# phonism/genrec

Hardware: AMD Instinct MI355X
Metric: train_samples_per_s (higher is better)
Workload: dtype bf16; 1 GPU; model=tiger-amazon-beauty, global_batch=256, seq_len=61, parallelism=dp1, hip_graph=True

## Files before the change

csrc/bindings.cpp:

```cpp
#include <torch/extension.h>

namespace genrec {

std::vector<torch::Tensor> rms_norm_fwd(torch::Tensor x, torch::Tensor w,
                                        double eps, bool t5_style);
std::vector<torch::Tensor> rms_norm_bwd(torch::Tensor dy, torch::Tensor x,
                                        torch::Tensor w, torch::Tensor inv_rms,
                                        bool t5_style);
std::vector<torch::Tensor> l2norm_fwd(torch::Tensor x, double eps);
torch::Tensor l2norm_bwd(torch::Tensor dy, torch::Tensor x,
                         torch::Tensor inv_norm, double eps);

std::vector<torch::Tensor> attn_fwd(
    torch::Tensor q, torch::Tensor k, torch::Tensor v,
    c10::optional<torch::Tensor> bias, c10::optional<torch::Tensor> key_pad,
    c10::optional<torch::Tensor> add_mask,
    c10::optional<torch::Tensor> query_mask,
    double scale, bool causal, int64_t act, double dropout_p, int64_t seed,
    c10::optional<torch::Tensor> seed_dev);
std::vector<torch::Tensor> attn_bwd(
    torch::Tensor dout, torch::Tensor q, torch::Tensor k, torch::Tensor v,
    torch::Tensor p_saved, torch::Tensor drop_mask,
    c10::optional<torch::Tensor> query_mask,
    double scale, int64_t act, double dropout_p, int64_t seed,
    bool bias_grad, int64_t bias_dim);

std::vector<torch::Tensor> attn_fwd_mfma(
    torch::Tensor q, torch::Tensor k, torch::Tensor v,
    c10::optional<torch::Tensor> bias, c10::optional<torch::Tensor> key_pad,
    c10::optional<torch::Tensor> add_mask,
    c10::optional<torch::Tensor> query_mask,
    double scale, bool causal, int64_t act, double dropout_p, int64_t seed,
    c10::optional<torch::Tensor> seed_dev,
    c10::optional<torch::Tensor> bias_bucket);
std::vector<torch::Tensor> attn_bwd_mfma(
    torch::Tensor dout, torch::Tensor q, torch::Tensor k, torch::Tensor v,
    torch::Tensor p_saved, torch::Tensor drop_mask,
    c10::optional<torch::Tensor> query_mask,
    double scale, int64_t act, double dropout_p, int64_t seed,
    bool bias_grad, int64_t bias_dim,
    c10::optional<torch::Tensor> bias_bucket, int64_t n_buckets);

std::vector<torch::Tensor> hstu_attn_fwd(
    torch::Tensor q, torch::Tensor k, torch::Tensor v,
    torch::Tensor pos_bucket, torch::Tensor pos_table,
    c10::optional<torch::Tensor> time_table,
    c10::optional<torch::Tensor> timestamps,
    c10::optional<torch::Tensor> key_pad);
std::vector<torch::Tensor> hstu_attn_bwd(
    torch::Tensor dout, torch::Tensor q, torch::Tensor k, torch::Tensor v,
    torch::Tensor s_saved, torch::Tensor pos_bucket,
    c10::optional<torch::Tensor> timestamps,
    int64_t n_pos, int64_t n_time);

std::vector<torch::Tensor> softmax_ce_fwd(torch::Tensor logits,
                                          torch::Tensor targets,
                                          int64_t ignore_index);
torch::Tensor softmax_ce_bwd(torch::Tensor dloss, torch::Tensor logits,
                             torch::Tensor targets, torch::Tensor lse,
                             torch::Tensor n_valid, int64_t ignore_index);
std::vector<torch::Tensor> lce_inplace(torch::Tensor logits,
                                       torch::Tensor targets,
                                       torch::Tensor inv_n,
                                       int64_t ignore_index, int64_t slices);
int64_t lce_pick_slices(int64_t R, int64_t V);

std::vector<torch::Tensor> sqdist_argmin(torch::Tensor x,
                                         torch::Tensor codebook);
torch::Tensor embedding_fwd(torch::Tensor weight, torch::Tensor indices);
torch::Tensor embedding_bwd(torch::Tensor dy, torch::Tensor indices,
                            int64_t num_weights, int64_t padding_idx);
std::vector<torch::Tensor> dropout_add_fwd(
    torch::Tensor x, torch::Tensor residual, double p, int64_t seed,
    c10::optional<torch::Tensor> seed_dev);
// ... 49 lines not shown
    torch::Tensor out, torch::Tensor lse,
    c10::optional<torch::Tensor> key_pad, double scale, bool causal);

torch::Tensor beam_attn_fwd(torch::Tensor q, torch::Tensor k_pre,
                            torch::Tensor v_pre,
                            c10::optional<torch::Tensor> pre_pad,
                            torch::Tensor k_suf, torch::Tensor v_suf,
                            torch::Tensor anc, int64_t t, double scale,
                            int64_t splits);
int64_t beam_attn_pick_splits(int64_t B, int64_t Hkv, int64_t rows,
                              int64_t Lp);

}

PYBIND11_MODULE(TORCH_EXTENSION_NAME, m) {
  m.def("rms_norm_fwd", &genrec::rms_norm_fwd, "fused RMSNorm forward");
  m.def("rms_norm_bwd", &genrec::rms_norm_bwd, "fused RMSNorm backward");
  m.def("l2norm_fwd", &genrec::l2norm_fwd, "fused L2Norm forward");
  m.def("l2norm_bwd", &genrec::l2norm_bwd, "fused L2Norm backward");
  m.def("attn_fwd", &genrec::attn_fwd, "fused attention forward");
  m.def("attn_bwd", &genrec::attn_bwd, "fused attention backward");
  m.def("attn_fwd_mfma", &genrec::attn_fwd_mfma, "MFMA attention forward",
        py::arg("q"), py::arg("k"), py::arg("v"), py::arg("bias"),
        py::arg("key_pad"), py::arg("add_mask"), py::arg("query_mask"),
        py::arg("scale"), py::arg("causal"), py::arg("act"),
        py::arg("dropout_p"), py::arg("seed"), py::arg("seed_dev"),
        py::arg("bias_bucket") = py::none());
  m.def("attn_bwd_mfma", &genrec::attn_bwd_mfma, "MFMA attention backward",
        py::arg("dout"), py::arg("q"), py::arg("k"), py::arg("v"),
        py::arg("p_saved"), py::arg("drop_mask"), py::arg("query_mask"),
        py::arg("scale"), py::arg("act"), py::arg("dropout_p"),
        py::arg("seed"), py::arg("bias_grad"), py::arg("bias_dim"),
        py::arg("bias_bucket") = py::none(),
        py::arg("n_buckets") = 0);
  m.def("hstu_attn_fwd", &genrec::hstu_attn_fwd, "HSTU fused attention fwd");
  m.def("hstu_attn_bwd", &genrec::hstu_attn_bwd, "HSTU fused attention bwd");
  m.def("softmax_ce_fwd", &genrec::softmax_ce_fwd, "fused CE forward");
  m.def("softmax_ce_bwd", &genrec::softmax_ce_bwd, "fused CE backward");
  m.def("lce_inplace", &genrec::lce_inplace,
        "in-place CE fwd+bwd over a logits chunk (lce_stats + lce_grad)",
        py::arg("logits"), py::arg("targets"), py::arg("inv_n"),
        py::arg("ignore_index"), py::arg("slices") = 0);
  m.def("lce_pick_slices", &genrec::lce_pick_slices,
        "column slices per row chosen for an [R, V] chunk");
  m.def("sqdist_argmin", &genrec::sqdist_argmin, "L2 dist + argmin");
  m.def("embedding_fwd", &genrec::embedding_fwd, "embedding gather");
  m.def("embedding_bwd", &genrec::embedding_bwd, "embedding scatter-add bwd");
  m.def("dropout_add_fwd", &genrec::dropout_add_fwd, "residual+dropout fwd");
  m.def("relu_dropout_fwd", &genrec::relu_dropout_fwd, "dropout(relu) fwd");
  m.def("plain_dropout_fwd", &genrec::plain_dropout_fwd,
        "graph-replay-safe plain dropout fwd");
  m.def("colsum", &genrec::colsum,
        "deterministic replay-safe column sum (bias grads)");
  m.def("chunk_sum", &genrec::chunk_sum,
        "small-row-count column sum (split-K dW partials)");
  m.def("layer_norm_fwd", &genrec::layer_norm_fwd, "fused LayerNorm fwd");
  m.def("layer_norm_bwd", &genrec::layer_norm_bwd, "fused LayerNorm bwd");
  m.def("dropout_fuse_bwd", &genrec::dropout_fuse_bwd, "fused dropout bwd");
  m.def("dropout_add_rms_norm_fwd", &genrec::dropout_add_rms_norm_fwd,
        "fused residual+dropout -> RMSNorm fwd -> (h, n, mask, inv_rms)");
  m.def("dropout_add_rms_norm_bwd", &genrec::dropout_add_rms_norm_bwd,
        "fused RMSNorm bwd + dh add + dropout bwd -> (t, dy, dw)");
  m.def("topk_hit_ranks", &genrec::topk_hit_ranks, "first-match ranks");
  m.def("fused_adamw", &genrec::fused_adamw,
        "fused flat AdamW step (device lr/scale/step scalars)");
  m.def("skinny_gemm", &genrec::skinny_gemm,
        "tall-skinny linear fwd GEMM (bf16, fp32 accum)");
// ... 19 lines not shown
```

csrc/kernels/attention_mfma.hip:

```cpp

#include <torch/extension.h>
#include <ATen/hip/HIPContext.h>

#include "../core/mfma_tile.h"

namespace genrec {

torch::Tensor colsum(torch::Tensor x);

template <bool IS_SILU>
__global__ void __launch_bounds__(256, 5)
attn_fwd_mfma_kernel(
    const __hip_bfloat16* __restrict__ q,
    const __hip_bfloat16* __restrict__ k,
    const __hip_bfloat16* __restrict__ v,
    const void* __restrict__ bias,
    const int* __restrict__ bias_bucket,
    const bool* __restrict__ key_pad,
    const float* __restrict__ add_mask,
    const float* __restrict__ query_mask,
    __hip_bfloat16* __restrict__ out,
    float* __restrict__ p_saved,
    unsigned char* __restrict__ drop_mask,
    const unsigned int* __restrict__ seed_dev,
    int B, int H, int Lq, int Lk, int D, int n_buckets,
    int64_t q_sb, int64_t q_sh, int64_t q_sl,
    int64_t k_sb, int64_t k_sh, int64_t k_sl,
    int64_t v_sb, int64_t v_sh, int64_t v_sl,
    int64_t o_sb, int64_t o_sh, int64_t o_sl,
    float scale, int bias_dim, bool bias_bf16, bool causal,
    float dropout_p, unsigned int seed, int q_tile) {
  if (seed_dev) seed += *seed_dev;
  const float* bias_f = reinterpret_cast<const float*>(bias);
  const __hip_bfloat16* bias_b = reinterpret_cast<const __hip_bfloat16*>(bias);
  const int bh = blockIdx.x;
  const int b = bh / H, h = bh % H;
  const int q0 = blockIdx.y * q_tile;

  extern __shared__ __attribute__((aligned(16))) char smem[];
  char* qs = smem;
  char* ks = qs + TILE * 128;
// ... 279 lines not shown
  float da[2][4], ad[2][4];
#pragma unroll
  for (int fi = 0; fi < 2; ++fi) {
#pragma unroll
    for (int r = 0; r < 4; ++r) {
      int i = strip + row_grp + r;
      int j = (fbase + fi) * 16 + col_base;
      bool ok = (i < Lq) && (j < Lk);
      float p = pv[fi][r];
      float m = 1.f;
      if (!IS_SILU && ok) {
        if (query_mask) m *= qm_v[r];
        if (dropout_p > 0.f) m *= dm_v[fi][r] ? inv_keep : 0.f;
      }
      da[fi][r] = ok ? acc[fi][r] * (IS_SILU ? 1.f : m) : 0.f;
      ad[fi][r] = IS_SILU ? (ok ? p * sigmoidf_dev(p) : 0.f) : p * m;
    }
  }

  float ds[2][4];
  if (IS_SILU) {
#pragma unroll
    for (int fi = 0; fi < 2; ++fi)
#pragma unroll
      for (int r = 0; r < 4; ++r) {
        float s = pv[fi][r];
        float sg = sigmoidf_dev(s);
        ds[fi][r] = da[fi][r] * sg * (1.f + s * (1.f - sg));
      }
  } else {
    float part[4];
#pragma unroll
    for (int r = 0; r < 4; ++r)
      part[r] = grp16_sum(da[0][r] * pv[0][r] + da[1][r] * pv[1][r]);
    if (col_base == 0) {
#pragma unroll
      for (int r = 0; r < 4; ++r)
        dotbuf[half * TILE + strip + row_grp + r] = part[r];
    }
    __syncthreads();
#pragma unroll
    for (int r = 0; r < 4; ++r) {
      float dot_r = dotbuf[strip + row_grp + r] +
                    dotbuf[TILE + strip + row_grp + r];
#pragma unroll
      for (int fi = 0; fi < 2; ++fi)
        ds[fi][r] = pv[fi][r] * (da[fi][r] - dot_r);
    }
  }

  const int i0 = strip + row_grp;
#pragma unroll
  for (int fi = 0; fi < 2; ++fi) {
    short4v dpack, apack;
#pragma unroll
    for (int r = 0; r < 4; ++r) {
      int i = i0 + r;
      int j = (fbase + fi) * 16 + col_base;
      float dval = (i < Lq && j < Lk) ? ds[fi][r] : 0.f;
      float aval = (i < Lq && j < Lk) ? ad[fi][r] : 0.f;
      dpack[r] = bf16_bits(dval * scale);
      apack[r] = bf16_bits(aval);
      if (ds_saved && i < Lq && j < Lk) {
        ds_saved[idx4(b, h, i, j, H, Lq, Lk)] = __float2bfloat16(dval);
      }
      if (dtab_partial && i < Lq && j < Lk) {
        atomicAdd(&tab_lds[bias_bucket[(int64_t)i * Lk + j]], dval);
// ... 32 lines not shown
              __float2bfloat16(accq[fi][r]);
        }
      }
    }
  }

  {
    float4v acck[2] = {{0.f, 0.f, 0.f, 0.f}, {0.f, 0.f, 0.f, 0.f}};
    float4v accv[2] = {{0.f, 0.f, 0.f, 0.f}, {0.f, 0.f, 0.f, 0.f}};
#pragma unroll
    for (int fi = 0; fi < 2; ++fi) {
      if (fbase + fi >= nfrag_d) break;
      for (int kk = 0; kk < TILE; kk += 32) {
        short8v a1 = frag_load<true>(dst, strip, kk, lane);
        short8v b1 = frag_load_tr(qs, kk, (fbase + fi) * 16, lane);
        acck[fi] = mfma_bf16(a1, b1, acck[fi]);
        short8v a2 = frag_load<true>(adt, strip, kk, lane);
        short8v b2 = frag_load_tr(dos, kk, (fbase + fi) * 16, lane);
        accv[fi] = mfma_bf16(a2, b2, accv[fi]);
      }
    }
#pragma unroll
    for (int fi = 0; fi < 2; ++fi) {
      if (fbase + fi >= nfrag_d) break;
#pragma unroll
      for (int r = 0; r < 4; ++r) {
        int j = strip + row_grp + r;
        int d = (fbase + fi) * 16 + col_base;
        if (j < Lk && d < D) {
          dk_out[(int64_t)b * dk_sb + h * dk_sh + j * dk_sl + d] =
              __float2bfloat16(acck[fi][r]);
          dv_out[(int64_t)b * dv_sb + h * dv_sh + j * dv_sl + d] =
              __float2bfloat16(accv[fi][r]);
        }
      }
    }
  }
}

constexpr int BS_CH = 16;

__global__ void batch_sum1_kernel(const __hip_bfloat16* __restrict__ in,
                                  float* __restrict__ tmp,
                                  int B, int64_t inner) {
  int64_t tid = (int64_t)blockIdx.x * blockDim.x + threadIdx.x;
  if (tid >= (int64_t)BS_CH * inner) return;
  int64_t j = tid % inner;
  int chunk = (int)(tid / inner);
  float acc = 0.f;
  for (int b = chunk; b < B; b += BS_CH)
    acc += to_f32(in[(int64_t)b * inner + j]);
  tmp[(int64_t)chunk * inner + j] = acc;
}

__global__ void batch_sum2_kernel(const float* __restrict__ tmp,
                                  float* __restrict__ out, int64_t inner) {
  int64_t j = (int64_t)blockIdx.x * blockDim.x + threadIdx.x;
  if (j >= inner) return;
  float acc = 0.f;
#pragma unroll
  for (int r = 0; r < BS_CH; ++r) acc += tmp[(int64_t)r * inner + j];
  out[j] = acc;
}


std::vector<torch::Tensor> attn_fwd_mfma(
    torch::Tensor q, torch::Tensor k, torch::Tensor v,
    c10::optional<torch::Tensor> bias, c10::optional<torch::Tensor> key_pad,
    c10::optional<torch::Tensor> add_mask,
    c10::optional<torch::Tensor> query_mask,
    double scale, bool causal, int64_t act, double dropout_p, int64_t seed,
    c10::optional<torch::Tensor> seed_dev,
    c10::optional<torch::Tensor> bias_bucket) {
  TORCH_CHECK(q.scalar_type() == torch::kBFloat16);
  const int B = q.size(0), H = q.size(1), Lq = q.size(2), D = q.size(3);
  const int Lk = k.size(2);
  TORCH_CHECK(Lk <= TILE && D <= TILE && D % 32 == 0);
  TORCH_CHECK(q.stride(3) == 1 && k.stride(3) == 1 && v.stride(3) == 1,
              "attn_fwd_mfma: innermost (D) stride must be 1");
  auto out = torch::empty_like(q);
  auto p_saved = torch::empty({B, H, Lq, Lk},
                              q.options().dtype(torch::kFloat32));
  torch::Tensor dmask;
  if (dropout_p > 0) {
    dmask = torch::empty({B, H, Lq, Lk}, q.options().dtype(torch::kUInt8));
  } else {
    dmask = torch::empty({0}, q.options().dtype(torch::kUInt8));
  }
  torch::Tensor bias_c, bucket_c;
  int bias_dim = 0;
  bool bias_bf16 = false;
  int n_buckets = 0;
  if (bias_bucket.has_value()) {
    TORCH_CHECK(bias.has_value() &&
                bias->scalar_type() == torch::kFloat32);
    bias_c = bias->contiguous();
    bucket_c = bias_bucket->to(torch::kInt32).contiguous();
    n_buckets = (int)(bias_c.numel() / H);
  } else if (bias.has_value()) {
    TORCH_CHECK(bias->scalar_type() == torch::kFloat32 ||
                bias->scalar_type() == torch::kBFloat16);
    bias_c = bias->contiguous();
    bias_dim = bias_c.dim();
    bias_bf16 = bias_c.scalar_type() == torch::kBFloat16;
  }
  torch::Tensor am_f, qm_f;
  if (add_mask.has_value()) am_f = add_mask->to(torch::kFloat32).contiguous();
  if (query_mask.has_value())
    qm_f = query_mask->to(torch::kFloat32).contiguous();

  const int q_tile = TILE;
  dim3 block(256);
  dim3 grid(B * H, (Lq + q_tile - 1) / q_tile);
  size_t smem = 4 * TILE * 128;
  auto stream = at::cuda::getCurrentHIPStream();

#define LAUNCH_FWD_MFMA(SILU)                                                  \
  hipLaunchKernelGGL((attn_fwd_mfma_kernel<SILU>), grid, block, smem, stream,  \
      reinterpret_cast<const __hip_bfloat16*>(q.data_ptr()),                   \
      reinterpret_cast<const __hip_bfloat16*>(k.data_ptr()),                   \
      reinterpret_cast<const __hip_bfloat16*>(v.data_ptr()),                   \
      (bias_dim || n_buckets) ? bias_c.data_ptr() : nullptr,                   \
      n_buckets ? bucket_c.data_ptr<int>() : nullptr,                          \
      key_pad.has_value() ? key_pad->data_ptr<bool>() : nullptr,               \
      add_mask.has_value() ? am_f.data_ptr<float>() : nullptr,                 \
      query_mask.has_value() ? qm_f.data_ptr<float>() : nullptr,               \
      reinterpret_cast<__hip_bfloat16*>(out.data_ptr()),                       \
      p_saved.data_ptr<float>(),                                               \
      dropout_p > 0 ? dmask.data_ptr<unsigned char>() : nullptr,               \
      seed_dev.has_value()                                                     \
          ? reinterpret_cast<const unsigned int*>(seed_dev->data_ptr())        \
          : nullptr,                                                           \
      B, H, Lq, Lk, D, n_buckets,                                              \
      q.stride(0), q.stride(1), q.stride(2),                                   \
      k.stride(0), k.stride(1), k.stride(2),                                   \
      v.stride(0), v.stride(1), v.stride(2),                                   \
      out.stride(0), out.stride(1), out.stride(2),                             \
      (float)scale, bias_dim, bias_bf16, causal,                               \
      (float)dropout_p, (unsigned int)seed, q_tile)

  if (act == 0) LAUNCH_FWD_MFMA(false);
  else LAUNCH_FWD_MFMA(true);
#undef LAUNCH_FWD_MFMA
  return {out, p_saved, dmask};
}

std::vector<torch::Tensor> attn_bwd_mfma(
    torch::Tensor dout, torch::Tensor q, torch::Tensor k, torch::Tensor v,
    torch::Tensor p_saved, torch::Tensor drop_mask,
    c10::optional<torch::Tensor> query_mask,
    double scale, int64_t act, double dropout_p, int64_t seed,
    bool bias_grad, int64_t bias_dim,
    c10::optional<torch::Tensor> bias_bucket, int64_t n_buckets) {
  (void)seed;
  const int B = q.size(0), H = q.size(1), Lq = q.size(2), D = q.size(3);
  const int Lk = k.size(2);
  TORCH_CHECK(Lq <= TILE && Lk <= TILE && D % 32 == 0);
  TORCH_CHECK(dout.stride(3) == 1 && q.stride(3) == 1 && k.stride(3) == 1 &&
                  v.stride(3) == 1,
              "attn_bwd_mfma: innermost (D) stride must be 1");
  auto dq = torch::empty_like(q);
  auto dk = torch::empty_like(k);
  auto dv = torch::empty_like(v);
  torch::Tensor ds_saved, bucket_c, dtab_partial;
  __hip_bfloat16* ds_ptr = nullptr;
  const bool table_mode = bias_grad && bias_bucket.has_value();
  if (table_mode) {
    bucket_c = bias_bucket->to(torch::kInt32).contiguous();
    dtab_partial = torch::empty({(int64_t)B * H, n_buckets},
                                q.options().dtype(torch::kFloat32));
  } else if (bias_grad) {
    ds_saved = torch::empty({B, H, Lq, Lk},
                            q.options().dtype(torch::kBFloat16));
    ds_ptr = reinterpret_cast<__hip_bfloat16*>(ds_saved.data_ptr());
  }
  torch::Tensor qm_f;
  if (query_mask.has_value())
    qm_f = query_mask->to(torch::kFloat32).contiguous();
  dim3 block(512);
  dim3 grid(B * H);
  size_t smem = 6 * TILE * 128 + 2 * TILE * sizeof(float)
      + (table_mode ? (size_t)n_buckets * sizeof(float) : 0);
  auto stream = at::cuda::getCurrentHIPStream();

#define LAUNCH_BWD_DS(SILU)                                                    \
  hipLaunchKernelGGL((attn_bwd_ds_kernel<SILU>), grid, block, smem, stream,    \
      reinterpret_cast<const __hip_bfloat16*>(dout.data_ptr()),                \
      reinterpret_cast<const __hip_bfloat16*>(q.data_ptr()),                   \
      reinterpret_cast<const __hip_bfloat16*>(k.data_ptr()),                   \
      reinterpret_cast<const __hip_bfloat16*>(v.data_ptr()),                   \
      p_saved.data_ptr<float>(),                                               \
      query_mask.has_value() ? qm_f.data_ptr<float>() : nullptr,               \
      dropout_p > 0 ? drop_mask.data_ptr<unsigned char>() : nullptr,           \
      reinterpret_cast<__hip_bfloat16*>(dq.data_ptr()),                        \
      reinterpret_cast<__hip_bfloat16*>(dk.data_ptr()),                        \
      reinterpret_cast<__hip_bfloat16*>(dv.data_ptr()), ds_ptr,                \
      table_mode ? bucket_c.data_ptr<int>() : nullptr,                         \
      table_mode ? dtab_partial.data_ptr<float>() : nullptr,                   \
      (int)n_buckets,                                                          \
      B, H, Lq, Lk, D,                                                         \
      dout.stride(0), dout.stride(1), dout.stride(2),                          \
      q.stride(0), q.stride(1), q.stride(2),                                   \
      k.stride(0), k.stride(1), k.stride(2),                                   \
      v.stride(0), v.stride(1), v.stride(2),                                   \
      dq.stride(0), dq.stride(1), dq.stride(2),                                \
      dk.stride(0), dk.stride(1), dk.stride(2),                                \
      dv.stride(0), dv.stride(1), dv.stride(2),                                \
      (float)scale, (float)dropout_p)

  if (act == 0) LAUNCH_BWD_DS(false);
  else LAUNCH_BWD_DS(true);
#undef LAUNCH_BWD_DS

  torch::Tensor dbias;
  if (table_mode) {
    dbias = colsum(dtab_partial.view({B, (int64_t)H * n_buckets}));
  } else if (bias_grad) {
    if (bias_dim == 3) {
      const int64_t inner = (int64_t)H * Lq * Lk;
      dbias = torch::empty({H, Lq, Lk},
                           q.options().dtype(torch::kFloat32));
      auto tmp = torch::empty({16, inner},
                              q.options().dtype(torch::kFloat32));
      dim3 rblock(256);
      dim3 rgrid1((unsigned)((16 * inner + 255) / 256));
      hipLaunchKernelGGL(batch_sum1_kernel, rgrid1, rblock, 0, stream,
          reinterpret_cast<const __hip_bfloat16*>(ds_saved.data_ptr()),
          tmp.data_ptr<float>(), B, inner);
      dim3 rgrid2((unsigned)((inner + 255) / 256));
      hipLaunchKernelGGL(batch_sum2_kernel, rgrid2, rblock, 0, stream,
          tmp.data_ptr<float>(), dbias.data_ptr<float>(), inner);
    } else {
      dbias = ds_saved.to(torch::kFloat32);
    }
  } else {
    dbias = torch::empty({0}, q.options().dtype(torch::kFloat32));
  }
  return {dq, dk, dv, dbias};
}

}
```

genrec_amd/modules/transformer.py:

```python

from __future__ import annotations

import math
import os
from typing import Optional

import torch
from torch import Tensor, nn

from genrec_amd import ops
from genrec_amd.ops.linear import SplitKLinear
from genrec_amd.modules.norms import RMSNorm, T5RMSNorm


def relative_position_bucket(relative_positions: Tensor, num_buckets: int = 32,
                             max_distance: int = 128,
                             bidirectional: bool = True) -> Tensor:
    ret = -relative_positions
    if bidirectional:
        num_buckets //= 2
        sign = (ret < 0).long()
        ret = ret.abs()
    else:
        ret = torch.clamp_min(ret, 0)
# ... 61 lines not shown
        return ops.embedding(self.rel_bias.weight, idx).view(
            self.n_heads, q_len, k_len)

    def _bucket_map(self, q_len: int, k_len: int, device) -> Tensor:
        key = ("bm", q_len, k_len, str(device))
        bm = self._bucket_cache.get(key)
        if bm is None:
            ctx = torch.arange(q_len, device=device)[:, None]
            mem = torch.arange(k_len, device=device)[None, :]
            bm = relative_position_bucket(
                mem - ctx, self.num_relative_buckets, self.max_distance,
                bidirectional=True).to(torch.int32).contiguous()
            self._bucket_cache[key] = bm
        return bm

    def _split(self, x: Tensor) -> Tensor:
        b, l, _ = x.shape
        return x.view(b, l, self.n_heads, self.head_dim).transpose(1, 2)

    def forward(self, query: Tensor, key: Optional[Tensor] = None,
                value: Optional[Tensor] = None,
                attn_mask: Optional[Tensor] = None,
                key_padding_mask: Optional[Tensor] = None,
                kv_cache: Optional[dict] = None) -> Tensor:
        if self.is_cross_attention:
            if kv_cache is not None and "k" in kv_cache:
                k, v = kv_cache["k"], kv_cache["v"]
            else:
                k, v = self._split(self.k(key)), self._split(self.v(value))
                if kv_cache is not None:
                    kv_cache["k"], kv_cache["v"] = k, v
        else:
            qkv = self.qkv(query)
            q_flat, k, v = qkv.chunk(3, dim=-1)
            k, v = self._split(k), self._split(v)
            if kv_cache is not None:
                if "k" in kv_cache:
                    k = torch.cat([kv_cache["k"], k], dim=2)
                    v = torch.cat([kv_cache["v"], v], dim=2)
                kv_cache["k"], kv_cache["v"] = k, v
            q = self._split(q_flat)
            return self._attend(q, k, v, attn_mask, key_padding_mask)
        q = self._split(self.q(query))
        return self._attend(q, k, v, attn_mask, key_padding_mask)

    def _attend(self, q: Tensor, k: Tensor, v: Tensor,
                attn_mask: Optional[Tensor],
                key_padding_mask: Optional[Tensor]) -> Tensor:

        bias = None
        bias_table = bias_bucket = None
        if self.rel_bias is not None:
            if os.environ.get("GENREC_ATTN_TABLE_BIAS", "0") == "1" \
                    and q.is_cuda:
                bias_table = self.rel_bias.weight.view(-1)
                bm = self._bucket_map(k.size(2), k.size(2), q.device)
                if q.size(2) != k.size(2):
                    bm = bm[k.size(2) - q.size(2):, :].contiguous()
                bias_bucket = bm
            else:
                bias = self.compute_bias(k.size(2), k.size(2), q.device)
                if q.size(2) != k.size(2):
                    bias = bias[:, k.size(2) - q.size(2):, :]

        out = ops.t5_attention(
            q, k, v, bias, key_padding_mask, attn_mask, self.scale,
# ... 175 lines not shown
```

genrec_amd/ops/__init__.py:

```python

from __future__ import annotations

import os

import torch

_EXT = None
_EXT_ERR: Exception | None = None


def _load_ext():
    global _EXT, _EXT_ERR
    if _EXT is not None or _EXT_ERR is not None:
        return _EXT
    try:
        from genrec_amd import _C

        _EXT = _C
    except ImportError as e:
        _EXT_ERR = e
        _EXT = None
    return _EXT


# ... 3 lines not shown
        raise RuntimeError(
            "genrec_amd HIP extension (genrec_amd._C) is not built. "
            "Run `python setup.py build_ext --inplace` (gfx950). "
            f"Import error: {_EXT_ERR}"
        )
    return m


def has_ext() -> bool:
    return _load_ext() is not None


def _force_eager() -> bool:
    return os.environ.get("GENREC_AMD_FORCE_EAGER", "0") == "1"


def use_hip(*tensors: torch.Tensor) -> bool:
    if _force_eager():
        return False
    if not tensors or not tensors[0].is_cuda:
        return False
    ext()
    return True


from genrec_amd.ops import eager
from genrec_amd.ops.norms import (
    layer_norm, rms_norm, l2norm_op, swish_layer_norm,
)
from genrec_amd.ops.attention import (
    fused_attention,
    sasrec_attention,
    t5_attention,
    hstu_pointwise_attention,
    hstu_fused_attention,
    gqa_flash_attention,
    beam_decode_attention,
    beam_decode_supported,
)
from genrec_amd.ops.quantize import residual_quantize_step
from genrec_amd.ops.losses import (
    softmax_ce, tied_softmax_ce, summed_ce, linear_cross_entropy,
)
from genrec_amd.ops.metrics import topk_hit_ranks
from genrec_amd.ops.embedding import embedding
from genrec_amd.ops.fused import (
    dropout_add, dropout_add_rms_norm, plain_dropout, relu_dropout,
)

__all__ = [
    "ext",
    "has_ext",
    "use_hip",
    "eager",
    "rms_norm",
    "l2norm_op",
    "swish_layer_norm",
    "layer_norm",
    "fused_attention",
    "sasrec_attention",
    "t5_attention",
    "hstu_pointwise_attention",
    "hstu_fused_attention",
    "gqa_flash_attention",
    "beam_decode_attention",
    "beam_decode_supported",
    "residual_quantize_step",
    "softmax_ce",
    "tied_softmax_ce",
    "summed_ce",
    "linear_cross_entropy",
    "topk_hit_ranks",
    "embedding",
    "dropout_add",
    "dropout_add_rms_norm",
    "plain_dropout",
    "relu_dropout",
]
```

genrec_amd/ops/attention.py:

```python

from __future__ import annotations

import os
from typing import Optional

import torch
from torch import Tensor

from genrec_amd.ops import eager

_ACT_SOFTMAX = 0
_ACT_SILU = 1


def _kernel_available(name: str, *tensors: Tensor) -> bool:
    from genrec_amd import ops

    if not ops.use_hip(*tensors):
        return False
    return hasattr(ops.ext(), name)


_seed_counters = {}
_call_salt = [0]
# ... 43 lines not shown
        out, probs, dmask = fwd(
            q, k, v, bias, key_pad_mask, additive_mask, query_mask,
            scale, causal, act, dropout_p if training else 0.0, seed,
            seed_dev,
        )
        ctx.use_mfma = use_mfma
        ctx.save_for_backward(q, k, v, probs, dmask,
                              query_mask if query_mask is not None else torch.empty(0))
        ctx.meta = (scale, causal, act, dropout_p if training else 0.0, seed,
                    bias is not None and bias.requires_grad,
                    bias.dim() if bias is not None else 0,
                    bias.dtype if bias is not None else None)
        return out

    @staticmethod
    def backward(ctx, dout):
        from genrec_amd import ops

        q, k, v, probs, dmask, query_mask = ctx.saved_tensors
        (scale, causal, act, dropout_p, seed, bias_grad, bias_dim,
         bias_dtype) = ctx.meta
        bwd = ops.ext().attn_bwd_mfma if ctx.use_mfma else ops.ext().attn_bwd
        if not (ctx.use_mfma and dout.stride(-1) == 1):
            dout = dout.contiguous()
        dq, dk, dv, dbias = bwd(
            dout, q, k, v, probs, dmask,
            query_mask if query_mask.numel() else None,
            scale, act, dropout_p, seed, bias_grad, bias_dim,
        )
        if bias_grad and dbias.dtype != bias_dtype:
            dbias = dbias.to(bias_dtype)
        return (dq, dk, dv, dbias if bias_grad else None,
                None, None, None, None, None, None, None, None)


class _FusedAttnTableBiasFn(torch.autograd.Function):

    @staticmethod
    def forward(ctx, q, k, v, bias_table, bias_bucket, key_pad_mask,
                additive_mask, query_mask, scale, causal, dropout_p,
                training):
        from genrec_amd import ops

        q = q if q.stride(-1) == 1 else q.contiguous()
        k = k if k.stride(-1) == 1 else k.contiguous()
        v = v if v.stride(-1) == 1 else v.contiguous()
        table_f = bias_table.float()
        seed_dev = None
        seed = 0
        if dropout_p > 0 and training:
            seed = _call_seed()
            seed_dev = _seed_counter(q.device)
        out, probs, dmask = ops.ext().attn_fwd_mfma(
            q, k, v, table_f, key_pad_mask, additive_mask, query_mask,
            scale, causal, 0, dropout_p if training else 0.0, seed,
            seed_dev, bias_bucket)
        ctx.save_for_backward(
            q, k, v, probs, dmask,
            query_mask if query_mask is not None else torch.empty(0),
            bias_bucket)
        ctx.meta = (scale, dropout_p if training else 0.0,
                    bias_table.requires_grad,
                    bias_table.numel() // q.size(1), bias_table.dtype)
        return out

    @staticmethod
# ... 331 lines not shown
```

Baseline: 54330 samples/s.

## Add small-Lq wave-per-head attention kernels and packed QKV self-attention path

```diff
diff --git a/csrc/bindings.cpp b/csrc/bindings.cpp
--- a/csrc/bindings.cpp
+++ b/csrc/bindings.cpp
@@ -39,7 +39,10 @@
     c10::optional<torch::Tensor> query_mask,
     double scale, int64_t act, double dropout_p, int64_t seed,
     bool bias_grad, int64_t bias_dim,
-    c10::optional<torch::Tensor> bias_bucket, int64_t n_buckets);
+    c10::optional<torch::Tensor> bias_bucket, int64_t n_buckets,
+    c10::optional<torch::Tensor> dqkv_out);
+std::string attn_mfma_path(int64_t Lq, int64_t Lk, int64_t D, int64_t act,
+                           bool table_mode, bool backward);
 
 std::vector<torch::Tensor> hstu_attn_fwd(
     torch::Tensor q, torch::Tensor k, torch::Tensor v,
@@ -155,7 +158,14 @@
         py::arg("scale"), py::arg("act"), py::arg("dropout_p"),
         py::arg("seed"), py::arg("bias_grad"), py::arg("bias_dim"),
         py::arg("bias_bucket") = py::none(),
-        py::arg("n_buckets") = 0);
+        py::arg("n_buckets") = 0,
+        py::arg("dqkv_out") = py::none());
+  m.def("attn_mfma_path", &genrec::attn_mfma_path,
+        "kernel family attn_fwd_mfma (attn_bwd_mfma: backward=True) runs "
+        "for a shape: "
+        "\"smallq\" or \"tile64\"",
+        py::arg("Lq"), py::arg("Lk"), py::arg("D"), py::arg("act") = 0,
+        py::arg("table_mode") = false, py::arg("backward") = false);
   m.def("hstu_attn_fwd", &genrec::hstu_attn_fwd, "HSTU fused attention fwd");
   m.def("hstu_attn_bwd", &genrec::hstu_attn_bwd, "HSTU fused attention bwd");
   m.def("softmax_ce_fwd", &genrec::softmax_ce_fwd, "fused CE forward");
diff --git a/csrc/kernels/attention_mfma.hip b/csrc/kernels/attention_mfma.hip
--- a/csrc/kernels/attention_mfma.hip
+++ b/csrc/kernels/attention_mfma.hip
@@ -7,6 +7,11 @@
 namespace genrec {
 
 torch::Tensor colsum(torch::Tensor x);
+
+__device__ __forceinline__ float jac_dot2(float a0, float b0, float a1,
+                                          float b1) {
+  return __builtin_fmaf(a0, b0, a1 * b1);
+}
 
 template <bool IS_SILU>
 __global__ void __launch_bounds__(256, 5)
@@ -352,7 +357,7 @@
     float part[4];
 #pragma unroll
     for (int r = 0; r < 4; ++r)
-      part[r] = grp16_sum(da[0][r] * pv[0][r] + da[1][r] * pv[1][r]);
+      part[r] = grp16_sum(jac_dot2(da[0][r], pv[0][r], da[1][r], pv[1][r]));
     if (col_base == 0) {
 #pragma unroll
       for (int r = 0; r < 4; ++r)
@@ -451,6 +456,485 @@
               __float2bfloat16(acck[fi][r]);
           dv_out[(int64_t)b * dv_sb + h * dv_sh + j * dv_sl + d] =
               __float2bfloat16(accv[fi][r]);
+        }
+      }
+    }
+  }
+}
+
+constexpr int SQ_HEADS = 2;
+constexpr int SQ_LQ = 16;
+constexpr int SQ_BWD_LK = 16;
+
+static inline int sq_rows32(int L) { return (L + 31) & ~31; }
+static inline size_t sq_fwd_lds(int Lk) {
+  return (size_t)(16 + 2 * sq_rows32(Lk)) * 128;
+}
+static inline size_t sq_bwd_lds(int Lk) {
+  return (size_t)(64 + 2 * sq_rows32(Lk)) * 128;
+}
+
+__device__ __forceinline__ void wave_lds_sync() {
+  __builtin_amdgcn_fence(__ATOMIC_ACQ_REL, "wavefront");
+  __builtin_amdgcn_wave_barrier();
+}
+
+template <int NF>
+__global__ void __launch_bounds__(64 * SQ_HEADS)
+attn_fwd_smallq_kernel(
+    const __hip_bfloat16* __restrict__ q,
+    const __hip_bfloat16* __restrict__ k,
+    const __hip_bfloat16* __restrict__ v,
+    const void* __restrict__ bias,
+    const bool* __restrict__ key_pad,
+    const float* __restrict__ add_mask,
+    const float* __restrict__ query_mask,
+    __hip_bfloat16* __restrict__ out,
+    float* __restrict__ p_saved,
+    unsigned char* __restrict__ drop_mask,
+    const unsigned int* __restrict__ seed_dev,
+    int B, int H, int Lq, int Lk, int D,
+    int64_t q_sb, int64_t q_sh, int64_t q_sl,
+    int64_t k_sb, int64_t k_sh, int64_t k_sl,
+    int64_t v_sb, int64_t v_sh, int64_t v_sl,
+    int64_t o_sb, int64_t o_sh, int64_t o_sl,
+    float scale, int bias_dim, bool bias_bf16, bool causal,
+    float dropout_p, unsigned int seed) {
+  const int lane = threadIdx.x & 63;
+  const int wid = __builtin_amdgcn_readfirstlane(threadIdx.x >> 6);
+  const int bh = blockIdx.x * SQ_HEADS + wid;
+  if (bh >= B * H) return;
+  if (seed_dev) seed += *seed_dev;
+  const float* bias_f = reinterpret_cast<const float*>(bias);
+  const __hip_bfloat16* bias_b = reinterpret_cast<const __hip_bfloat16*>(bias);
+  const int b = bh / H, h = bh % H;
+  constexpr int nf = NF;
+  constexpr int kr = (NF + 1) / 2 * 32;
+
+  extern __shared__ __attribute__((aligned(16))) char smem[];
+  char* qs = smem + (size_t)wid * (16 + 2 * kr) * 128;
+  char* ks = qs + 16 * 128;
+  char* vs = ks + kr * 128;
+  char* pt = ks;
+
+  const int col_base = frag_col(lane);
+  const int row_grp = frag_row0(lane);
+
+  const int st_row = lane >> 3;
+  const int st_d0 = (lane & 7) * 8;
+  short8v qq8[2], kk8[kr / 8], vv8[kr / 8];
+#pragma unroll
+  for (int c = 0; c < 2; ++c) {
+    int row = c * 8 + st_row;
+    qq8[c] = load8(q, (int64_t)b * q_sb + h * q_sh + row * q_sl + st_d0,
+                   row < Lq && st_d0 < D);
+  }
+#pragma unroll
+  for (int c = 0; c < kr / 8; ++c) {
+    int row = c * 8 + st_row;
+    kk8[c] = load8(k, (int64_t)b * k_sb + h * k_sh + row * k_sl + st_d0,
+                   row < Lk && st_d0 < D);
+    vv8[c] = load8(v, (int64_t)b * v_sb + h * v_sh + row * v_sl + st_d0,
+                   row < Lk && st_d0 < D);
+  }
+
+  float bias_v[4][4], am_v[4][4];
+  bool kp_v[4];
+#pragma unroll
+  for (int f = 0; f < 4; ++f) {
+    int j = f * 16 + col_base;
+    kp_v[f] = (key_pad && f < nf && j < Lk) ? key_pad[(int64_t)b * Lk + j] : false;
+#pragma unroll
+    for (int r = 0; r < 4; ++r) {
+      int i = row_grp + r;
+      bool ok = (f < nf) && (i < Lq) && (j < Lk);
+      float bv = 0.f, av = 0.f;
+      if (ok) {
+        if (bias_dim) {
+          int64_t bi = (bias_dim == 3) ? ((int64_t)h * Lq + i) * Lk + j
+                                       : idx4(b, h, i, j, H, Lq, Lk);
+          bv = bias_bf16 ? to_f32(bias_b[bi]) : bias_f[bi];
+        }
+        if (add_mask) av = add_mask[(int64_t)i * Lk + j];
+      }
+      bias_v[f][r] = bv;
+      am_v[f][r] = av;
+    }
+  }
+
+#pragma unroll
+  for (int c = 0; c < 2; ++c)
+    tile_store(qs, c * 8 + st_row, st_d0, qq8[c]);
+#pragma unroll
+  for (int c = 0; c < kr / 8; ++c) {
+    if (c * 8 < nf * 16) tile_store(ks, c * 8 + st_row, st_d0, kk8[c]);
+    tile_store<true>(vs, c * 8 + st_row, st_d0, vv8[c]);
+  }
+  wave_lds_sync();
+
+  const float inv_keep = dropout_p > 0.f ? 1.0f / (1.0f - dropout_p) : 1.0f;
+
+  float4v acc[4] = {{0.f, 0.f, 0.f, 0.f}, {0.f, 0.f, 0.f, 0.f},
+                    {0.f, 0.f, 0.f, 0.f}, {0.f, 0.f, 0.f, 0.f}};
+#pragma unroll
+  for (int f = 0; f < 4; ++f) {
+    if (f >= nf) break;
+    for (int kk = 0; kk < D; kk += 32) {
+      short8v a = frag_load(qs, 0, kk, lane);
+      short8v bfr = frag_load(ks, f * 16, kk, lane);
+      acc[f] = mfma_bf16(a, bfr, acc[f]);
+    }
+  }
+
+  float s_val[4][4];
+#pragma unroll
+  for (int f = 0; f < 4; ++f) {
+#pragma unroll
+    for (int r = 0; r < 4; ++r) {
+      int i = row_grp + r;
+      int j = f * 16 + col_base;
+      float s = acc[f][r];
+      bool ok = (f < nf) && (i < Lq) && (j < Lk);
+      if (ok) {
+        s *= scale;
+        if (bias_dim) s += bias_v[f][r];
+        if (causal && j > i) s = NEG_BIG;
+        if (kp_v[f]) s = NEG_BIG;
+        if (add_mask) s += am_v[f][r];
+      } else {
+        s = -INFINITY;
+      }
+      s_val[f][r] = s;
+    }
+  }
+
+  float p_val[4][4];
+#pragma unroll
+  for (int r = 0; r < 4; ++r) {
+    float m = grp16_max(fmaxf(fmaxf(s_val[0][r], s_val[1][r]),
+                              fmaxf(s_val[2][r], s_val[3][r])));
+    float sum = 0.f;
+#pragma unroll
+    for (int f = 0; f < 4; ++f) {
+      float e = (s_val[f][r] == -INFINITY) ? 0.f
+                                           : __expf(s_val[f][r] - m);
+      p_val[f][r] = e;
+      sum += e;
+    }
+    sum = grp16_sum(sum);
+    float inv = (sum > 0.f) ? 1.0f / sum : 0.f;
+#pragma unroll
+    for (int f = 0; f < 4; ++f) p_val[f][r] *= inv;
+  }
+
+  wave_lds_sync();
+
+#pragma unroll
+  for (int f = 0; f < 4; ++f) {
+    if (f * 16 >= kr) break;
+    short4v ppack;
+#pragma unroll
+    for (int r = 0; r < 4; ++r) {
+      int i = row_grp + r;
+      int j = f * 16 + col_base;
+      float p = p_val[f][r];
+      if (f < nf && i < Lq && j < Lk) {
+        p_saved[idx4(b, h, i, j, H, Lq, Lk)] = p;
+        if (query_mask) p *= query_mask[(int64_t)b * Lq + i];
+        if (dropout_p > 0.f) {
+          unsigned long long gidx = idx4(b, h, i, j, H, Lq, Lk);
+          bool keep = (hash_rng(seed, gidx) & 0xFFFFFF) >=
+                      (unsigned int)(dropout_p * 16777216.0f);
+          drop_mask[gidx] = keep;
+          p = keep ? p * inv_keep : 0.f;
+        }
+      } else {
+        p = 0.f;
+      }
+      ppack[r] = bf16_bits(p);
+    }
+    tile_store<true>(pt, f * 16 + col_base, row_grp, ppack);
+  }
+  wave_lds_sync();
+
+  float4v acc2[4] = {{0.f, 0.f, 0.f, 0.f}, {0.f, 0.f, 0.f, 0.f},
+                     {0.f, 0.f, 0.f, 0.f}, {0.f, 0.f, 0.f, 0.f}};
+  const int nfrag_d = (D + 15) / 16;
+#pragma unroll
+  for (int f = 0; f < 4; ++f) {
+    if (f >= nfrag_d) break;
+    for (int kk = 0; kk < kr; kk += 32) {
+      short8v a = frag_load_tr(pt, kk, 0, lane);
+      short8v bfr = frag_load_tr(vs, kk, f * 16, lane);
+      acc2[f] = mfma_bf16(a, bfr, acc2[f]);
+    }
+  }
+#pragma unroll
+  for (int f = 0; f < 4; ++f) {
+    if (f >= nfrag_d) break;
+#pragma unroll
+    for (int r = 0; r < 4; ++r) {
+      int i = row_grp + r;
+      int d = f * 16 + col_base;
+      if (i < Lq && d < D) {
+        out[(int64_t)b * o_sb + h * o_sh + i * o_sl + d] =
+            __float2bfloat16(acc2[f][r]);
+      }
+    }
+  }
+}
+
+template <int NF>
+__global__ void __launch_bounds__(64 * SQ_HEADS)
+attn_bwd_smallq_kernel(
+    const __hip_bfloat16* __restrict__ dout,
+    const __hip_bfloat16* __restrict__ q,
+    const __hip_bfloat16* __restrict__ k,
+    const __hip_bfloat16* __restrict__ v,
+    const float* __restrict__ p_saved,
+    const float* __restrict__ query_mask,
+    const unsigned char* __restrict__ drop_mask,
+    __hip_bfloat16* __restrict__ dq_out,
+    __hip_bfloat16* __restrict__ dk_out,
+    __hip_bfloat16* __restrict__ dv_out,
+    __hip_bfloat16* __restrict__ ds_saved,
+    int B, int H, int Lq, int Lk, int D,
+    int64_t do_sb, int64_t do_sh, int64_t do_sl,
+    int64_t q_sb, int64_t q_sh, int64_t q_sl,
+    int64_t k_sb, int64_t k_sh, int64_t k_sl,
+    int64_t v_sb, int64_t v_sh, int64_t v_sl,
+    int64_t dq_sb, int64_t dq_sh, int64_t dq_sl,
+    int64_t dk_sb, int64_t dk_sh, int64_t dk_sl,
+    int64_t dv_sb, int64_t dv_sh, int64_t dv_sl,
+    float scale, float dropout_p) {
+  const int lane = threadIdx.x & 63;
+  const int wid = __builtin_amdgcn_readfirstlane(threadIdx.x >> 6);
+  const int bh = blockIdx.x * SQ_HEADS + wid;
+  if (bh >= B * H) return;
+  const int b = bh / H, h = bh % H;
+  constexpr int nf = NF;
+  constexpr int kr = (NF + 1) / 2 * 32;
+
+  extern __shared__ __attribute__((aligned(16))) char smem[];
+  char* dos = smem + (size_t)wid * (64 + 2 * kr) * 128;
+  char* qs = dos + 32 * 128;
+  char* ks = qs + 32 * 128;
+  char* vs = ks + kr * 128;
+  char* adt = vs;
+  char* dst = vs;
+
+  const int col_base = frag_col(lane);
+  const int row_grp = frag_row0(lane);
+
+  const int st_row = lane >> 3;
+  const int st_d0 = (lane & 7) * 8;
+  short8v dd8[2], qq8[2], kk8[kr / 8], vv8[kr / 8];
+#pragma unroll
+  for (int c = 0; c < 2; ++c) {
+    int row = c * 8 + st_row;
+    const bool q_ok = row < Lq && st_d0 < D;
+    dd8[c] = load8(dout, (int64_t)b * do_sb + h * do_sh + row * do_sl + st_d0,
+                   q_ok);
+    qq8[c] = load8(q, (int64_t)b * q_sb + h * q_sh + row * q_sl + st_d0,
+                   q_ok);
+  }
+#pragma unroll
+  for (int c = 0; c < kr / 8; ++c) {
+    int row = c * 8 + st_row;
+    const bool k_ok = row < Lk && st_d0 < D;
+    vv8[c] = load8(v, (int64_t)b * v_sb + h * v_sh + row * v_sl + st_d0,
+                   k_ok);
+    kk8[c] = load8(k, (int64_t)b * k_sb + h * k_sh + row * k_sl + st_d0,
+                   k_ok);
+  }
+
+  float pv[4][4], qm_v[4];
+  unsigned char dm_v[4][4];
+#pragma unroll
+  for (int r = 0; r < 4; ++r) {
+    int i = row_grp + r;
+    qm_v[r] = (query_mask && i < Lq) ? query_mask[(int64_t)b * Lq + i] : 1.f;
+#pragma unroll
+    for (int f = 0; f < 4; ++f) {
+      int j = f * 16 + col_base;
+      bool ok = (f < nf) && (i < Lq) && (j < Lk);
+      pv[f][r] = ok ? p_saved[idx4(b, h, i, j, H, Lq, Lk)] : 0.f;
+      dm_v[f][r] = (dropout_p > 0.f && ok)
+                       ? drop_mask[idx4(b, h, i, j, H, Lq, Lk)] : 0;
+    }
+  }
+
+#pragma unroll
+  for (int c = 0; c < 2; ++c) {
+    tile_store<true>(dos, c * 8 + st_row, st_d0, dd8[c]);
+    tile_store<true>(qs, c * 8 + st_row, st_d0, qq8[c]);
+    tile_store<true>(dos, 16 + c * 8 + st_row, st_d0, short8v{});
+    tile_store<true>(qs, 16 + c * 8 + st_row, st_d0, short8v{});
+  }
+#pragma unroll
+  for (int c = 0; c < kr / 8; ++c) {
+    if (c * 8 < nf * 16) tile_store<true>(vs, c * 8 + st_row, st_d0, vv8[c]);
+    tile_store<true>(ks, c * 8 + st_row, st_d0, kk8[c]);
+  }
+  wave_lds_sync();
+
+  const float inv_keep = dropout_p > 0.f ? 1.0f / (1.0f - dropout_p) : 1.0f;
+
+  float4v acc[4] = {{0.f, 0.f, 0.f, 0.f}, {0.f, 0.f, 0.f, 0.f},
+                    {0.f, 0.f, 0.f, 0.f}, {0.f, 0.f, 0.f, 0.f}};
+#pragma unroll
+  for (int f = 0; f < 4; ++f) {
+    if (f >= nf) break;
+    for (int kk = 0; kk < D; kk += 32) {
+      short8v a = frag_load<true>(dos, 0, kk, lane);
+      short8v bfr = frag_load<true>(vs, f * 16, kk, lane);
+      acc[f] = mfma_bf16(a, bfr, acc[f]);
+    }
+  }
+
+  float da[4][4], ad[4][4];
+#pragma unroll
+  for (int f = 0; f < 4; ++f) {
+#pragma unroll
+    for (int r = 0; r < 4; ++r) {
+      int i = row_grp + r;
+      int j = f * 16 + col_base;
+      bool ok = (f < nf) && (i < Lq) && (j < Lk);
+      float p = pv[f][r];
+      float m = 1.f;
+      if (ok) {
+        if (query_mask) m *= qm_v[r];
+        if (dropout_p > 0.f) m *= dm_v[f][r] ? inv_keep : 0.f;
+      }
+      da[f][r] = ok ? acc[f][r] * m : 0.f;
+      ad[f][r] = p * m;
+    }
+  }
+
+  float ds[4][4];
+#pragma unroll
+  for (int r = 0; r < 4; ++r) {
+    float part0 = grp16_sum(jac_dot2(da[0][r], pv[0][r], da[1][r], pv[1][r]));
+    float part1 = grp16_sum(jac_dot2(da[2][r], pv[2][r], da[3][r], pv[3][r]));
+    float dot_r = part0 + part1;
+#pragma unroll
+    for (int f = 0; f < 4; ++f)
+      ds[f][r] = pv[f][r] * (da[f][r] - dot_r);
+  }
+
+  wave_lds_sync();
+  const short4v zero4 = {0, 0, 0, 0};
+#pragma unroll
+  for (int f = 0; f < 4; ++f) {
+    if (f * 16 >= kr) break;
+    short4v apack;
+#pragma unroll
+    for (int r = 0; r < 4; ++r) {
+      int i = row_grp + r;
+      int j = f * 16 + col_base;
+      float aval = (f < nf && i < Lq && j < Lk) ? ad[f][r] : 0.f;
+      apack[r] = bf16_bits(aval);
+    }
+    int j = f * 16 + col_base;
+    tile_store<true>(adt, j, row_grp, apack);
+    tile_store<true>(adt, j, 16 + row_grp, zero4);
+  }
+  wave_lds_sync();
+
+  const int nfrag_d = (D + 15) / 16;
+  for (int js = 0; js < nf; ++js) {
+    float4v accv[4] = {{0.f, 0.f, 0.f, 0.f}, {0.f, 0.f, 0.f, 0.f},
+                       {0.f, 0.f, 0.f, 0.f}, {0.f, 0.f, 0.f, 0.f}};
+    short8v a2 = frag_load<true>(adt, js * 16, 0, lane);
+#pragma unroll
+    for (int f = 0; f < 4; ++f) {
+      if (f >= nfrag_d) break;
+      short8v b2 = frag_load_tr(dos, 0, f * 16, lane);
+      accv[f] = mfma_bf16(a2, b2, accv[f]);
+    }
+#pragma unroll
+    for (int f = 0; f < 4; ++f) {
+      if (f >= nfrag_d) break;
+#pragma unroll
+      for (int r = 0; r < 4; ++r) {
+        int j = js * 16 + row_grp + r;
+        int d = f * 16 + col_base;
+        if (j < Lk && d < D) {
+          dv_out[(int64_t)b * dv_sb + h * dv_sh + j * dv_sl + d] =
+              __float2bfloat16(accv[f][r]);
+        }
+      }
+    }
+  }
+
+  wave_lds_sync();
+#pragma unroll
+  for (int f = 0; f < 4; ++f) {
+    if (f * 16 >= kr) break;
+    short4v dpack;
+#pragma unroll
+    for (int r = 0; r < 4; ++r) {
+      int i = row_grp + r;
+      int j = f * 16 + col_base;
+      float dval = (f < nf && i < Lq && j < Lk) ? ds[f][r] : 0.f;
+      dpack[r] = bf16_bits(dval * scale);
+      if (ds_saved && f < nf && i < Lq && j < Lk) {
+        ds_saved[idx4(b, h, i, j, H, Lq, Lk)] = __float2bfloat16(dval);
+      }
+    }
+    int j = f * 16 + col_base;
+    tile_store<true>(dst, j, row_grp, dpack);
+    tile_store<true>(dst, j, 16 + row_grp, zero4);
+  }
+  wave_lds_sync();
+
+  {
+    float4v accq[4] = {{0.f, 0.f, 0.f, 0.f}, {0.f, 0.f, 0.f, 0.f},
+                       {0.f, 0.f, 0.f, 0.f}, {0.f, 0.f, 0.f, 0.f}};
+#pragma unroll
+    for (int f = 0; f < 4; ++f) {
+      if (f >= nfrag_d) break;
+      for (int kk = 0; kk < kr; kk += 32) {
+        short8v a = frag_load_tr(dst, kk, 0, lane);
+        short8v bfr = frag_load_tr(ks, kk, f * 16, lane);
+        accq[f] = mfma_bf16(a, bfr, accq[f]);
+      }
+    }
+#pragma unroll
+    for (int f = 0; f < 4; ++f) {
+      if (f >= nfrag_d) break;
+#pragma unroll
+      for (int r = 0; r < 4; ++r) {
+        int i = row_grp + r;
+        int d = f * 16 + col_base;
+        if (i < Lq && d < D) {
+          dq_out[(int64_t)b * dq_sb + h * dq_sh + i * dq_sl + d] =
+              __float2bfloat16(accq[f][r]);
+        }
+      }
+    }
+  }
+
+  for (int js = 0; js < nf; ++js) {
+    float4v acck[4] = {{0.f, 0.f, 0.f, 0.f}, {0.f, 0.f, 0.f, 0.f},
+                       {0.f, 0.f, 0.f, 0.f}, {0.f, 0.f, 0.f, 0.f}};
+    short8v a1 = frag_load<true>(dst, js * 16, 0, lane);
+#pragma unroll
+    for (int f = 0; f < 4; ++f) {
+      if (f >= nfrag_d) break;
+      short8v b1 = frag_load_tr(qs, 0, f * 16, lane);
+      acck[f] = mfma_bf16(a1, b1, acck[f]);
+    }
+#pragma unroll
+    for (int f = 0; f < 4; ++f) {
+      if (f >= nfrag_d) break;
+#pragma unroll
+      for (int r = 0; r < 4; ++r) {
+        int j = js * 16 + row_grp + r;
+        int d = f * 16 + col_base;
+        if (j < Lk && d < D) {
+          dk_out[(int64_t)b * dk_sb + h * dk_sh + j * dk_sl + d] =
+              __float2bfloat16(acck[f][r]);
         }
       }
     }
@@ -482,6 +966,21 @@
   out[j] = acc;
 }
 
+
+static bool smallq_applies(int64_t Lq, int64_t Lk, int64_t D, int64_t act,
+                           bool table_mode, bool backward) {
+  if (Lq < 1 || Lq > SQ_LQ || Lk < 1 || Lk > (backward ? SQ_BWD_LK : TILE) ||
+      D > TILE || D % 32 != 0 || act != 0 || table_mode)
+    return false;
+  const char* knob = std::getenv("GENREC_ATTN_SMALLQ");
+  return !(knob && knob[0] == '0' && knob[1] == '\0');
+}
+
+std::string attn_mfma_path(int64_t Lq, int64_t Lk, int64_t D, int64_t act,
+                           bool table_mode, bool backward) {
+  return smallq_applies(Lq, Lk, D, act, table_mode, backward) ? "smallq"
+                                                              : "tile64";
+}
 
 std::vector<torch::Tensor> attn_fwd_mfma(
     torch::Tensor q, torch::Tensor k, torch::Tensor v,
@@ -528,11 +1027,44 @@
   if (query_mask.has_value())
     qm_f = query_mask->to(torch::kFloat32).contiguous();
 
+  auto stream = at::cuda::getCurrentHIPStream();
+
+  if (smallq_applies(Lq, Lk, D, act, bias_bucket.has_value(), false)) {
+    dim3 sq_block(64 * SQ_HEADS);
+    dim3 sq_grid((B * H + SQ_HEADS - 1) / SQ_HEADS);
+    auto kern = attn_fwd_smallq_kernel<1>;
+    if (Lk > 48) kern = attn_fwd_smallq_kernel<4>;
+    else if (Lk > 32) kern = attn_fwd_smallq_kernel<3>;
+    else if (Lk > 16) kern = attn_fwd_smallq_kernel<2>;
+    hipLaunchKernelGGL(kern, sq_grid, sq_block,
+        SQ_HEADS * sq_fwd_lds(Lk), stream,
+        reinterpret_cast<const __hip_bfloat16*>(q.data_ptr()),
+        reinterpret_cast<const __hip_bfloat16*>(k.data_ptr()),
+        reinterpret_cast<const __hip_bfloat16*>(v.data_ptr()),
+        bias_dim ? bias_c.data_ptr() : nullptr,
+        key_pad.has_value() ? key_pad->data_ptr<bool>() : nullptr,
+        add_mask.has_value() ? am_f.data_ptr<float>() : nullptr,
+        query_mask.has_value() ? qm_f.data_ptr<float>() : nullptr,
+        reinterpret_cast<__hip_bfloat16*>(out.data_ptr()),
+        p_saved.data_ptr<float>(),
+        dropout_p > 0 ? dmask.data_ptr<unsigned char>() : nullptr,
+        seed_dev.has_value()
+            ? reinterpret_cast<const unsigned int*>(seed_dev->data_ptr())
+            : nullptr,
+        B, H, Lq, Lk, D,
+        q.stride(0), q.stride(1), q.stride(2),
+        k.stride(0), k.stride(1), k.stride(2),
+        v.stride(0), v.stride(1), v.stride(2),
+        out.stride(0), out.stride(1), out.stride(2),
+        (float)scale, bias_dim, bias_bf16, causal,
+        (float)dropout_p, (unsigned int)seed);
+    return {out, p_saved, dmask};
+  }
+
   const int q_tile = TILE;
   dim3 block(256);
   dim3 grid(B * H, (Lq + q_tile - 1) / q_tile);
   size_t smem = 4 * TILE * 128;
-  auto stream = at::cuda::getCurrentHIPStream();
 
 #define LAUNCH_FWD_MFMA(SILU)                                                  \
   hipLaunchKernelGGL((attn_fwd_mfma_kernel<SILU>), grid, block, smem, stream,  \
@@ -570,7 +1102,8 @@
     c10::optional<torch::Tensor> query_mask,
     double scale, int64_t act, double dropout_p, int64_t seed,
     bool bias_grad, int64_t bias_dim,
-    c10::optional<torch::Tensor> bias_bucket, int64_t n_buckets) {
+    c10::optional<torch::Tensor> bias_bucket, int64_t n_buckets,
+    c10::optional<torch::Tensor> dqkv_out) {
   (void)seed;
   const int B = q.size(0), H = q.size(1), Lq = q.size(2), D = q.size(3);
   const int Lk = k.size(2);
@@ -578,9 +1111,25 @@
   TORCH_CHECK(dout.stride(3) == 1 && q.stride(3) == 1 && k.stride(3) == 1 &&
                   v.stride(3) == 1,
               "attn_bwd_mfma: innermost (D) stride must be 1");
-  auto dq = torch::empty_like(q);
-  auto dk = torch::empty_like(k);
-  auto dv = torch::empty_like(v);
+  torch::Tensor dq, dk, dv;
+  if (dqkv_out.has_value()) {
+    TORCH_CHECK(Lq == Lk, "attn_bwd_mfma: dqkv_out needs Lq == Lk");
+    TORCH_CHECK(dqkv_out->scalar_type() == torch::kBFloat16 &&
+                    dqkv_out->is_contiguous() && dqkv_out->dim() == 3 &&
+                    dqkv_out->size(0) == B && dqkv_out->size(1) == Lq &&
+                    dqkv_out->size(2) == (int64_t)3 * H * D &&
+                    dqkv_out->device() == q.device(),
+                "attn_bwd_mfma: dqkv_out must be contiguous bf16 "
+                "[B, L, 3*H*D]");
+    auto parts = dqkv_out->view({B, Lq, 3, H, D});
+    dq = parts.select(2, 0).transpose(1, 2);
+    dk = parts.select(2, 1).transpose(1, 2);
+    dv = parts.select(2, 2).transpose(1, 2);
+  } else {
+    dq = torch::empty_like(q);
+    dk = torch::empty_like(k);
+    dv = torch::empty_like(v);
+  }
   torch::Tensor ds_saved, bucket_c, dtab_partial;
   __hip_bfloat16* ds_ptr = nullptr;
   const bool table_mode = bias_grad && bias_bucket.has_value();
@@ -596,11 +1145,40 @@
   torch::Tensor qm_f;
   if (query_mask.has_value())
     qm_f = query_mask->to(torch::kFloat32).contiguous();
+  auto stream = at::cuda::getCurrentHIPStream();
+  const bool smallq =
+      smallq_applies(Lq, Lk, D, act, bias_bucket.has_value(), true);
   dim3 block(512);
   dim3 grid(B * H);
   size_t smem = 6 * TILE * 128 + 2 * TILE * sizeof(float)
       + (table_mode ? (size_t)n_buckets * sizeof(float) : 0);
-  auto stream = at::cuda::getCurrentHIPStream();
+
+  if (smallq) {
+    dim3 sq_block(64 * SQ_HEADS);
+    dim3 sq_grid((B * H + SQ_HEADS - 1) / SQ_HEADS);
+    static_assert(SQ_BWD_LK == 16, "one key strip: instance <1>");
+    hipLaunchKernelGGL(attn_bwd_smallq_kernel<1>, sq_grid, sq_block,
+        SQ_HEADS * sq_bwd_lds(Lk), stream,
+        reinterpret_cast<const __hip_bfloat16*>(dout.data_ptr()),
+        reinterpret_cast<const __hip_bfloat16*>(q.data_ptr()),
+        reinterpret_cast<const __hip_bfloat16*>(k.data_ptr()),
+        reinterpret_cast<const __hip_bfloat16*>(v.data_ptr()),
+        p_saved.data_ptr<float>(),
+        query_mask.has_value() ? qm_f.data_ptr<float>() : nullptr,
+        dropout_p > 0 ? drop_mask.data_ptr<unsigned char>() : nullptr,
+        reinterpret_cast<__hip_bfloat16*>(dq.data_ptr()),
+        reinterpret_cast<__hip_bfloat16*>(dk.data_ptr()),
+        reinterpret_cast<__hip_bfloat16*>(dv.data_ptr()), ds_ptr,
+        B, H, Lq, Lk, D,
+        dout.stride(0), dout.stride(1), dout.stride(2),
+        q.stride(0), q.stride(1), q.stride(2),
+        k.stride(0), k.stride(1), k.stride(2),
+        v.stride(0), v.stride(1), v.stride(2),
+        dq.stride(0), dq.stride(1), dq.stride(2),
+        dk.stride(0), dk.stride(1), dk.stride(2),
+        dv.stride(0), dv.stride(1), dv.stride(2),
+        (float)scale, (float)dropout_p);
+  }
 
 #define LAUNCH_BWD_DS(SILU)                                                    \
   hipLaunchKernelGGL((attn_bwd_ds_kernel<SILU>), grid, block, smem, stream,    \
@@ -627,8 +1205,10 @@
       dv.stride(0), dv.stride(1), dv.stride(2),                                \
       (float)scale, (float)dropout_p)
 
-  if (act == 0) LAUNCH_BWD_DS(false);
-  else LAUNCH_BWD_DS(true);
+  if (!smallq) {
+    if (act == 0) LAUNCH_BWD_DS(false);
+    else LAUNCH_BWD_DS(true);
+  }
 #undef LAUNCH_BWD_DS
 
   torch::Tensor dbias;
diff --git a/genrec_amd/modules/transformer.py b/genrec_amd/modules/transformer.py
--- a/genrec_amd/modules/transformer.py
+++ b/genrec_amd/modules/transformer.py
@@ -117,6 +117,20 @@
                     kv_cache["k"], kv_cache["v"] = k, v
         else:
             qkv = self.qkv(query)
+            table_bias = self.rel_bias is not None and \
+                os.environ.get("GENREC_ATTN_TABLE_BIAS", "0") == "1"
+            if ops.packed_qkv_eligible(qkv, self.n_heads, attn_mask,
+                                       kv_cache, table_bias):
+                seq = qkv.size(1)
+                bias = None
+                if self.rel_bias is not None:
+                    bias = self.compute_bias(seq, seq, qkv.device)
+                out = ops.t5_self_attention_packed(
+                    qkv, self.n_heads, bias, key_padding_mask, attn_mask,
+                    self.scale, self.dropout_p, self.training)
+                out = out.transpose(1, 2).reshape(qkv.size(0), -1,
+                                                  self.d_model)
+                return self.o(out)
             q_flat, k, v = qkv.chunk(3, dim=-1)
             k, v = self._split(k), self._split(v)
             if kv_cache is not None:
diff --git a/genrec_amd/ops/__init__.py b/genrec_amd/ops/__init__.py
--- a/genrec_amd/ops/__init__.py
+++ b/genrec_amd/ops/__init__.py
@@ -59,6 +59,8 @@
     fused_attention,
     sasrec_attention,
     t5_attention,
+    t5_self_attention_packed,
+    packed_qkv_eligible,
     hstu_pointwise_attention,
     hstu_fused_attention,
     gqa_flash_attention,
@@ -87,6 +89,8 @@
     "fused_attention",
     "sasrec_attention",
     "t5_attention",
+    "t5_self_attention_packed",
+    "packed_qkv_eligible",
     "hstu_pointwise_attention",
     "hstu_fused_attention",
     "gqa_flash_attention",
diff --git a/genrec_amd/ops/attention.py b/genrec_amd/ops/attention.py
--- a/genrec_amd/ops/attention.py
+++ b/genrec_amd/ops/attention.py
@@ -99,6 +99,97 @@
             dbias = dbias.to(bias_dtype)
         return (dq, dk, dv, dbias if bias_grad else None,
                 None, None, None, None, None, None, None, None)
+
+
+def _qkv_views(qkv: Tensor, n_heads: int):
+    b, l, w = qkv.shape
+    parts = qkv.view(b, l, 3, n_heads, w // (3 * n_heads))
+    return (parts[:, :, 0].transpose(1, 2), parts[:, :, 1].transpose(1, 2),
+            parts[:, :, 2].transpose(1, 2))
+
+
+class _PackedSelfAttnFn(torch.autograd.Function):
+
+    @staticmethod
+    def forward(ctx, qkv, n_heads, bias, key_pad_mask, additive_mask, scale,
+                dropout_p, training):
+        from genrec_amd import ops
+
+        qkv = qkv if qkv.is_contiguous() else qkv.contiguous()
+        q, k, v = _qkv_views(qkv, n_heads)
+        seed_dev = None
+        seed = 0
+        if dropout_p > 0 and training:
+            seed = _call_seed()
+            seed_dev = _seed_counter(qkv.device)
+        out, probs, dmask = ops.ext().attn_fwd_mfma(
+            q, k, v, bias, key_pad_mask, additive_mask, None,
+            scale, False, _ACT_SOFTMAX, dropout_p if training else 0.0, seed,
+            seed_dev,
+        )
+        ctx.save_for_backward(qkv, probs, dmask)
+        ctx.meta = (n_heads, scale, dropout_p if training else 0.0, seed,
+                    bias is not None and bias.requires_grad,
+                    bias.dim() if bias is not None else 0,
+                    bias.dtype if bias is not None else None)
+        return out
+
+    @staticmethod
+    def backward(ctx, dout):
+        from genrec_amd import ops
+
+        qkv, probs, dmask = ctx.saved_tensors
+        (n_heads, scale, dropout_p, seed, bias_grad, bias_dim,
+         bias_dtype) = ctx.meta
+        q, k, v = _qkv_views(qkv, n_heads)
+        if dout.stride(-1) != 1:
+            dout = dout.contiguous()
+        dqkv = torch.empty_like(qkv)
+        _, _, _, dbias = ops.ext().attn_bwd_mfma(
+            dout, q, k, v, probs, dmask, None,
+            scale, _ACT_SOFTMAX, dropout_p, seed, bias_grad, bias_dim,
+            None, 0, dqkv,
+        )
+        if bias_grad and dbias.dtype != bias_dtype:
+            dbias = dbias.to(bias_dtype)
+        return (dqkv, None, dbias if bias_grad else None,
+                None, None, None, None, None)
+
+
+def _packed_qkv_fits(qkv: Tensor, n_heads: int,
+                     additive_mask: Optional[Tensor], kv_cache: Optional[dict],
+                     table_bias: bool) -> bool:
+    if kv_cache is not None or table_bias or qkv.dim() != 3:
+        return False
+    if qkv.dtype != torch.bfloat16 or qkv.size(2) % (3 * n_heads) != 0:
+        return False
+    d = qkv.size(2) // (3 * n_heads)
+    if d % 32 != 0 or d > 64 or qkv.size(1) > 64 or qkv.size(1) < 1:
+        return False
+    return additive_mask is None or additive_mask.dim() == 2
+
+
+def packed_qkv_eligible(qkv: Tensor, n_heads: int,
+                        additive_mask: Optional[Tensor] = None,
+                        kv_cache: Optional[dict] = None,
+                        table_bias: bool = False) -> bool:
+    if not _packed_qkv_fits(qkv, n_heads, additive_mask, kv_cache,
+                            table_bias) or not qkv.is_cuda:
+        return False
+    for knob in ("GENREC_DISABLE_PACKED_QKV", "GENREC_DISABLE_ATTN",
+                 "GENREC_FORCE_FLASH", "GENREC_DISABLE_MFMA"):
+        if os.environ.get(knob, "0") == "1":
+            return False
+    return _kernel_available("attn_fwd_mfma", qkv)
+
+
+def t5_self_attention_packed(qkv, n_heads, bias, key_pad_mask, additive_mask,
+                             scale, dropout_p, training):
+    b = bias.contiguous() if bias is not None else None
+    kp = key_pad_mask.contiguous() if key_pad_mask is not None else None
+    am = additive_mask.contiguous() if additive_mask is not None else None
+    return _PackedSelfAttnFn.apply(qkv, n_heads, b, kp, am, scale, dropout_p,
+                                   training)
 
 
 class _FusedAttnTableBiasFn(torch.autograd.Function):
```

New measurement: 56810 samples/s (median of 6 runs). +4.6%, better.
